# ddiazdom/grlBWT

Measured on NVIDIA B200. Metric: input MB/s through the parse phase of the BCR BWT construction (all grammar rounds on device); whole construction: bwt_total, higher is better.
Workload: dtype u8

## Files before the change

grlbwt_b200/__init__.py:

```python
from .api import (GrlGpu, GrlGpuError, Round, Stats, build_bwt, build_bwt_file, build_bwt_packed, build_bwt_to, invert_rl_bwt, parse_rl_bwt, lib_gpu, lib_host,
                  selftest_compact, selftest_induce, selftest_scan, selftest_sort, FLAG_SMALL_TABLE,
                  FLAG_FORCE_SLOW_SCAN, FLAG_KEEP_DICT, FLAG_FORCE_UNCACHED, FLAG_SMALL_PILOT, FLAG_FORCE_DOUBLING, FLAG_FORCE_WALK,
                  FLAG_FORCE_JUMP, LIB_DIR, Slice)
```

grlbwt_b200/api.py:

```python
from __future__ import annotations

import ctypes as C
import os

import numpy as np

LIB_DIR = os.path.join(os.path.dirname(os.path.abspath(__file__)), "lib")
FLAG_SMALL_TABLE, FLAG_FORCE_SLOW_SCAN, FLAG_KEEP_DICT, FLAG_FORCE_UNCACHED, FLAG_SMALL_PILOT, FLAG_FORCE_DOUBLING = 1, 2, 4, 8, 16, 32
FLAG_FORCE_WALK, FLAG_FORCE_JUMP = 64, 128
CELL = {1: np.uint8, 2: np.uint16, 4: np.uint32, 8: np.uint64}


class GrlGpuError(RuntimeError):
    def __init__(self, status, msg):
        super().__init__(f"grlgpu status {status}: {msg}")
        self.status = status


class Stats(C.Structure):
    _fields_ = [(k, C.c_uint64) for k in ("n_syms", "n_strings", "longest_string", "min_sym", "max_sym", "max_sym_freq", "sep_sym")]


class Round(C.Structure):
    _fields_ = [(k, C.c_uint64) for k in ("round", "n_in", "n_strings", "parse_len", "n_phrases", "dict_syms", "max_freq", "alphabet",
# ... 60 lines not shown
        L.grlgpu_round.argtypes = [vp, C.POINTER(Round)]
        L.grlgpu_fetch_level.argtypes = [vp, vp, vp, vp, vp, vp]
        L.grlgpu_fetch_level_async.argtypes = [vp, vp, vp, vp, vp, vp]
        L.grlgpu_fetch_level32.argtypes = [vp, vp, vp, vp, vp, vp, C.c_int]
        L.grlgpu_fetch_wait.argtypes = [vp]
        L.grlgpu_level_checksum.argtypes = [vp, vp]
        L.grlgpu_fetch_parse.argtypes = [vp, vp]
        L.grlgpu_fetch_str_ptrs.argtypes = [vp, vp]
        L.grlgpu_fetch_dictionary.argtypes = [vp, vp, vp, vp, vp]
        L.grlgpu_strerror.restype = C.c_char_p
        L.grlgpu_strerror.argtypes = [C.c_int]
        L.grlgpu_last_error.restype = C.c_char_p
        L.grlgpu_last_error.argtypes = [vp]
        L.grlgpu_create_on_stream.argtypes = [C.POINTER(vp), C.c_int, u64, vp]
        L.grlgpu_profile_enable.argtypes = [vp, C.c_int]
        L.grlgpu_profile_reset.argtypes = [vp]
        L.grlgpu_launch_count.argtypes = [vp]
        L.grlgpu_launch_count.restype = u64
        L.grlgpu_profile_entry.argtypes = [vp, C.c_int, C.c_char_p, C.c_int, C.POINTER(u64), C.POINTER(C.c_double), C.POINTER(u64)]
        L.grlgpu_histogram.argtypes = [vp, vp]
        L.grlgpu_nccl_unique_id.argtypes = [vp]
        L.grlgpu_comm_create_nccl.argtypes = [C.POINTER(vp), vp, C.c_int, C.c_int, C.c_int]
        L.grlgpu_comm_create_ipc.argtypes = [C.POINTER(vp), C.c_char_p, C.c_int, C.c_int, C.c_int]
        L.grlgpu_can_peer.argtypes = [C.c_int, C.c_int]
        L.grlgpu_local_group_create.argtypes = [C.POINTER(vp), C.c_int]
        L.grlgpu_local_group_abort.argtypes = [vp]
        L.grlgpu_local_group_destroy.argtypes = [vp]
        L.grlgpu_comm_create_local.argtypes = [C.POINTER(vp), vp, C.c_int, C.c_int]
        L.grlgpu_comm_destroy.argtypes = [vp]
        L.grlgpu_comm_info.argtypes = [vp, C.POINTER(u64), C.POINTER(u64), C.POINTER(u64), C.c_char_p, C.c_int]
        L.grlgpu_comm_times.argtypes = [vp, C.POINTER(C.c_double), C.POINTER(C.c_double)]
        L.grlgpu_set_peers.argtypes = [vp, vp, C.c_int]
        L.grlgpu_mg_stats.argtypes = [vp, vp, C.POINTER(Stats)]
        L.grlgpu_mg_round.argtypes = [vp, vp, C.POINTER(Round)]
        L.grlgpu_mg_slice_info.argtypes = [vp, C.POINTER(Slice)]
        L.grlgpu_mg_fetch_slice.argtypes = [vp, vp, vp, vp, vp, vp, C.c_int, C.c_int]
        L.grlgpu_mg_slice_checksum.argtypes = [vp, vp]
        L.grlgpu_text_begin.argtypes = [vp, u64, C.c_int, u64]
        L.grlgpu_text_stage.argtypes = [vp, C.POINTER(vp), C.POINTER(u64)]
        L.grlgpu_text_commit.argtypes = [vp, u64]
        L.grlgpu_text_end.argtypes = [vp]
        L.grlgpu_level_park.argtypes = [vp, C.c_int, vp]
        L.grlgpu_copy_to_host.argtypes = [C.c_int, vp, vp, u64]
        L.grlgpu_invert.argtypes = [vp, vp, u64, C.c_int, u64, vp, u64, C.POINTER(Invert)]
        L.grlgpu_fm_load.argtypes = [vp, vp, u64, C.POINTER(FmInfo)]
        L.grlgpu_fm_count.argtypes = [vp, vp, vp, u64, C.c_int, vp, C.POINTER(FmQuery)]
        L.grlgpu_fm_locate.argtypes = [vp, vp, vp, u64, C.c_int, vp, vp, vp, u64, C.POINTER(FmQuery)]
        L.grlgpu_fm_approx_count.argtypes = [vp, vp, vp, u64, C.c_int, C.c_uint32, vp, vp, vp, u64, C.POINTER(FmApprox)]
        L.grlgpu_fm_approx_locate.argtypes = [vp, vp, vp, u64, C.c_int, C.c_uint32, vp, vp, vp, vp, u64, C.POINTER(FmApprox)]
        L.grlgpu_fm_extract.argtypes = [vp, vp, vp, vp, u64, C.c_int, vp, vp, u64, C.POINTER(FmExtract)]
        L.grlgpu_fm_drop.argtypes = [vp]
        L.grlgpu_selftest_scan.argtypes = [vp, u64, vp, vp]
        L.grlgpu_selftest_sort.argtypes = [vp, vp, u64, C.c_int]
        L.grlgpu_selftest_compact.argtypes = [vp, vp, u64, vp, vp]
        L.grlgpu_selftest_ipc_rendezvous.argtypes = [C.c_char_p, C.c_int, C.c_int, C.c_int]
        _gpu = L
    return _gpu


def lib_host():
    global _host
    if _host is None:
        lib_gpu()
        path = os.path.join(LIB_DIR, "libgrlbwt.so")
        if not os.path.exists(path):
            raise RuntimeError(f"{path} is missing: build it with `make -C grlbwt_b200`")
        L = C.CDLL(path)
        L.grlbwt_build.argtypes = [C.c_void_p, C.c_uint64, C.c_int, C.c_int, C.c_int, C.c_int, C.POINTER(BwtResult)]
        L.grlbwt_free_result.argtypes = [C.POINTER(BwtResult)]
        L.grlbwt_build_file.argtypes = [C.c_char_p, C.c_char_p, C.c_int, C.c_int, C.c_int, C.c_int]
        L.grlbwt_last_error.restype = C.c_char_p
        L.grlbwt_build_mg.argtypes = [C.c_void_p, C.c_uint64, C.c_int, C.c_void_p, C.c_int, C.c_int, C.c_int, C.c_int, C.POINTER(BwtResult)]
        L.grlbwt_build_to.argtypes = [C.c_void_p, C.c_uint64, C.c_int, C.c_void_p, C.c_int, C.c_int, C.c_int, C.c_void_p, C.c_void_p, C.c_uint64, C.POINTER(BwtResult)]
        L.grlbwt_build_packed.argtypes = [C.c_void_p, C.c_uint64, C.c_int, C.c_void_p, C.c_int, C.c_int, C.c_int, C.c_void_p, C.c_uint64, C.POINTER(C.c_uint64),
                                          C.POINTER(BwtResult)]
        L.grlbwt_last_digests.argtypes = [C.c_void_p, C.c_uint64]
        L.grlbwt_last_digests.restype = C.c_uint64
        L.grlbwt_last_exchange_bytes.restype = C.c_uint64
        L.grlbwt_last_comm.restype = C.c_char_p
        _host = L
    return _host


def _ptr(a):
    return None if a is None else a.ctypes.data_as(C.c_void_p)


def _carve(sizes, arena, offset):
    if arena is None:
        return [np.zeros(n, dt) for n, dt in sizes], None
    arrs, off = [], int(offset)
    for n, dt in sizes:
        nb = n * np.dtype(dt).itemsize
        off = (off + 15) & ~15
        if off + nb > arena.size:
            raise GrlGpuError(-1, "fetch arena too small")
        arrs.append(arena[off:off + nb].view(dt))
        off += nb
    return arrs, (off + 15) & ~15


class GrlGpu:

    def __init__(self, device: int = 0, flags: int = 0, stream: int = 0):
        self._L = lib_gpu()
        self._h = C.c_void_p()
# ... 435 lines not shown


def selftest_induce(levels, final_parse: np.ndarray, n_threads: int = 0):
    L = lib_host()
    n = len(levels)
    u64p, u8p = C.POINTER(C.c_uint64), C.POINTER(C.c_uint8)
    keep = []

    def arr(key, dt, ptype):
        out = (ptype * n)()
        for i, lv in enumerate(levels):
            a = np.ascontiguousarray(lv[key], dt)
            if a.size == 0:
                a = np.zeros(1, dt)
            keep.append(a)
            out[i] = a.ctypes.data_as(ptype)
        return out

    alph = np.array([lv["alphabet"] for lv in levels], np.uint64)
    tot = np.array([lv["tot"] for lv in levels], np.uint64)
    npre = np.array([len(lv["pre_sym"]) for lv in levels], np.uint64)
    fp = np.ascontiguousarray(final_parse, np.uint64)
    res = BwtResult()
    L.grlbwt_selftest_induce.argtypes = [C.c_int, C.c_void_p, C.c_void_p, C.POINTER(u64p), C.POINTER(u64p), C.POINTER(u8p), C.c_void_p,
                                         C.POINTER(u64p), C.POINTER(u64p), C.c_void_p, C.c_uint64, C.c_int, C.POINTER(BwtResult)]
    rc = L.grlbwt_selftest_induce(n, _ptr(alph), _ptr(tot), arr("rule_l", np.uint64, u64p), arr("rule_r", np.uint64, u64p),
                                  arr("has_hocc", np.uint8, u8p), _ptr(npre), arr("pre_sym", np.uint64, u64p), arr("pre_len", np.uint64, u64p),
                                  _ptr(fp), fp.size, n_threads, C.byref(res))
    if rc != 0:
        raise RuntimeError(L.grlbwt_last_error().decode())
    try:
        return (np.ctypeslib.as_array(res.syms, shape=(res.n_runs,)).copy(), np.ctypeslib.as_array(res.lens, shape=(res.n_runs,)).copy())
    finally:
        L.grlbwt_free_result(C.byref(res))


def selftest_scan(a: np.ndarray):
    a = np.ascontiguousarray(a, np.uint32)
    out, tot = np.zeros(a.size, np.uint64), np.zeros(1, np.uint64)
    rc = lib_gpu().grlgpu_selftest_scan(_ptr(a), a.size, _ptr(out), _ptr(tot))
    if rc != 0:
        raise GrlGpuError(rc, lib_gpu().grlgpu_strerror(rc).decode())
    return out, int(tot[0])


def selftest_sort(keys: np.ndarray, vals: np.ndarray, n_bits: int):
    k, v = np.ascontiguousarray(keys, np.uint64).copy(), np.ascontiguousarray(vals, np.uint32).copy()
    rc = lib_gpu().grlgpu_selftest_sort(_ptr(k), _ptr(v), k.size, n_bits)
    if rc != 0:
        raise GrlGpuError(rc, lib_gpu().grlgpu_strerror(rc).decode())
    return k, v


def selftest_compact(bits: np.ndarray, prev_bits, n_bits: int):
    b = np.ascontiguousarray(bits, np.uint32)
    pb = None if prev_bits is None else np.ascontiguousarray(prev_bits, np.uint32)
    out, cnt = np.zeros(max(1, n_bits), np.uint64), np.zeros(1, np.uint64)
    rc = lib_gpu().grlgpu_selftest_compact(_ptr(b), _ptr(pb), n_bits, _ptr(out), _ptr(cnt))
    if rc != 0:
        raise GrlGpuError(rc, lib_gpu().grlgpu_strerror(rc).decode())
    return out[: int(cnt[0])]
```

grlbwt_b200/csrc/grlgpu.cu:

```cuda
#include "../../include/grlgpu.h"
#include "util.cuh"
#include "primitives.cuh"
#include "parse_kernels.cuh"
#include "dict_kernels.cuh"
#include "comm.hpp"

#include <algorithm>
#include <cstring>
#include <memory>
#include <vector>

using namespace grl;


struct DevLevel {
    int sym_bytes = 4;
    u64 tot = 0, n_pre = 0;
    DevBuf<u8> rule_l, rule_r, has_hocc, pre_sym;
    DevBuf<u64> pre_len;
    bool present() const { return rule_l.p != nullptr; }
};

struct LevelView {
    int sym_bytes;
// ... 404 lines not shown
               R.einfo.p, (const u32*)voff.p, c->alphabet + 1, R.sym_bits, R.K, R.spare, R.keys.p, R.vals.p);
}

void refine_sort_groups(cudaStream_t st, const u64* nk, const u32* gflag, u64 nA, int key_bits, DevBuf<u32>& perm, DevBuf<u32>& flags) {
    perm.alloc(nA, st);
    flags.alloc(nA, st);
    if (nA == 0) return;
    DevBuf<u32> lflag(nA, st), lexcl(nA, st), cnt(1, st);
    GRL_LAUNCH("ext_local_sort", nA * 24, ext_local_sort_kernel, (unsigned)div_up(nA, LS_WIN), LS_THREADS, 0, st, nk, gflag, nA, perm.p, flags.p, lflag.p);
    exclusive_scan<u32, u32>(lflag.p, lexcl.p, nA, cnt.p, st);
    const u64 nLft = d2h_scalar(cnt.p, st);
    if (getenv("GRLGPU_TRACE")) fprintf(stderr, "[grlgpu]   refine sort: %llu active, %llu through the device-wide path\n", nA, nLft);
    if (nLft == 0) return;
    DevBuf<u32> lpos(nLft, st), lv(nLft, st), lv_alt(nLft, st), lg(nLft, st), gexcl(nLft, st), lf(nLft, st);
    DevBuf<u64> lk(nLft, st), lk_alt(nLft, st), lnk(nLft, st);
    GRL_LAUNCH("ext_left_gather", nA * 8 + nLft * 32, ext_left_gather_kernel, grid_for(nA, 256), 256, 0, st, lflag.p, lexcl.p, nk, gflag, nA, lpos.p, lk.p, lnk.p, lv.p, lg.p);
    exclusive_scan<u32, u32>(lg.p, gexcl.p, nLft, cnt.p, st);
    const u64 n_groups = d2h_scalar(cnt.p, st);
    u64 *kp = lk.p, *ka = lk_alt.p;
    u32 *vp = lv.p, *va = lv_alt.p;
    radix_sort_pairs(&kp, &vp, &ka, &va, nLft, key_bits, st);
    GRL_LAUNCH("ext_gid", nLft * 12, ext_gid_kernel, grid_for(nLft, 256), 256, 0, st, lg.p, gexcl.p, nLft);
    GRL_LAUNCH("ext_group_keys", nLft * 16, ext_group_keys_kernel, grid_for(nLft, 256), 256, 0, st, vp, gexcl.p, nLft, kp);
    radix_sort_pairs(&kp, &vp, &ka, &va, nLft, std::max(1, bit_width64(n_groups)), st);
    GRL_LAUNCH("ext_heads", nLft * 24, ext_heads_kernel, grid_for(nLft, 256), 256, 0, st, vp, kp, lnk.p, nLft, lf.p);
    GRL_LAUNCH("ext_left_scatter", nLft * 20, ext_left_scatter_kernel, grid_for(nLft, 256), 256, 0, st, lpos.p, vp, lf.p, nLft, perm.p, flags.p);
    GRL_CUDA(cudaStreamSynchronize(st));
}

template <class SymT>
void stage_dict(Round& R) {
    grlgpu_ctx* c = R.c;
    cudaStream_t st = R.st;
    const u64 nE = R.nE, A = c->alphabet;
    const SymT* D = (const SymT*)R.D_raw.p;
    IsSuffix isuf{c->is_suffix.p, c->sep, c->first};

    const bool ext_mode = R.ext_mode;
    const u64 nS = R.nS;
    const u64 n_words = div_up(nS, 32);
    DevBuf<u32> order_buf, head_bits(n_words, st);
    u64 G = 0;
    {
        DevBuf<u64> keys = std::move(R.keys), keys_alt(nS, st);
        DevBuf<u32> vals = std::move(R.vals), vals_alt(nS, st);
        const int sym_bits = R.sym_bits, K = R.K;
        if (!ext_mode) {
            keys.alloc(nS, st);
            vals.alloc(nS, st);
            GRL_LAUNCH("sfx_first_key", nE * (sizeof(SymT) + 4 + 12), (sfx_first_key_kernel<SymT>), grid_for(nE, 256), 256, 0, st, D, R.rem.p, nE, A + 1, sym_bits, K, keys.p, vals.p);
        }
        u64 *kp = keys.p, *ka = keys_alt.p;
        u32 *vp = vals.p, *va = vals_alt.p;
        radix_sort_pairs(&kp, &vp, &ka, &va, nS, std::min(64, sym_bits * K + R.spare), st);
        if (vp != vals.p) std::swap(vals, vals_alt);
        order_buf = std::move(vals);
        vals_alt.release();
        u32* order_w = order_buf.p;
        u64 nA = 0;
        DevBuf<u32> apos;
        if (ext_mode) {
            {
                DevBuf<u32> flags(nS, st), active_bits(n_words, st);
                GRL_LAUNCH("first_heads", nS * 12, first_heads_kernel, grid_for(nS, 256), 256, 0, st, kp, nS, sym_bits, R.spare, A + 1, flags.p, head_bits.p, active_bits.p);
                keys.release(); keys_alt.release();
                BitmapCompactor ac;
                nA = ac.count(active_bits.p, nS, st);
                apos.alloc(nA, st);
                if (nA) ac.write<u32>(nullptr, apos.p);
            }
            u64 dpt = (u64)K;
            while (nA > 0) {
                if (dpt > R.max_len + 1) throw Error(GRLGPU_ERR_STATE, "suffix refinement did not converge");
                DevBuf<u64> nk(nA, st);
                DevBuf<u32> ev(nA, st), gflag(nA, st), excl(nA, st), cnt(1, st), perm, flags;
                GRL_LAUNCH("ext_keys", nA * 32, (ext_keys_kernel<SymT>), grid_for(nA, 256), 256, 0, st, apos.p, order_w, D, R.rem.p, head_bits.p, nA, dpt, A + 1, sym_bits, K,
                           (u64*)nullptr, (u32*)nullptr, nk.p, ev.p, gflag.p);
                if (getenv("GRLGPU_TRACE")) fprintf(stderr, "[grlgpu] round %d refine: depth %llu, active %llu (of %llu sorted)\n", c->round + 1, dpt, nA, nS);
                refine_sort_groups(st, nk.p, gflag.p, nA, std::min(64, sym_bits * K), perm, flags);
                const u32* avp = perm.p;
                GRL_LAUNCH("ext_writeback", nA * 16, ext_writeback_kernel, grid_for(nA, 256), 256, 0, st, apos.p, avp, ev.p, flags.p, nA, order_w, head_bits.p);
                dpt += (u64)K;
                GRL_LAUNCH("ext_next", nA * 16, ext_next_kernel, grid_for(nA, 256), 256, 0, st, apos.p, avp, ev.p, head_bits.p, R.rem.p, nA, nS, dpt, flags.p);
                exclusive_scan<u32, u32>(flags.p, excl.p, nA, cnt.p, st);
                const u64 nA2 = d2h_scalar(cnt.p, st);
                DevBuf<u32> apos2(nA2, st);
                if (nA2) GRL_LAUNCH("compact_apos", nA * 12, compact_apos_kernel, grid_for(nA, 256), 256, 0, st, flags.p, excl.p, apos.p, nA, apos2.p);
                apos = std::move(apos2);
                nA = nA2;
            }
        } else {
        R.rank.alloc(nE, st);
        {
            DevBuf<u32> flags(nE, st), excl(nE, st), active_bits(n_words, st), gcount(1, st);
            GRL_LAUNCH("first_heads", nE * 12, first_heads_kernel, grid_for(nE, 256), 256, 0, st, kp, nE, sym_bits, 0, A + 1, flags.p, head_bits.p, active_bits.p);
            keys.release(); keys_alt.release();
            exclusive_scan<u32, u32>(flags.p, excl.p, nE, gcount.p, st);
            const u64 G0 = d2h_scalar(gcount.p, st);
            DevBuf<u32> head_pos(G0, st);
            GRL_LAUNCH("head_pos", nE * 8, head_pos_kernel, grid_for(nE, 256), 256, 0, st, flags.p, excl.p, (const u32*)nullptr, nE, head_pos.p);
            if (nE <= (1ull << 24)) {
                GRL_LAUNCH("assign_hrank", nE * 20, assign_hrank_kernel, grid_for(nE, 256), 256, 0, st, flags.p, excl.p, head_pos.p, order_w, nE, R.rank.p);
            } else {
                DevBuf<u32> pk(nE, st), pv(nE, st), pk2(nE, st), pv2(nE, st);
                GRL_LAUNCH("hrank_pairs", nE * 20, hrank_pairs_kernel, grid_for(nE, 256), 256, 0, st, flags.p, excl.p, head_pos.p, order_w, nE, pk.p, pv.p);
                u32 *k1 = pk.p, *v1 = pv.p, *k2 = pk2.p, *v2 = pv2.p;
                radix_partition_u32(&k1, &v1, &k2, &v2, nE, 24, st);
// ... 1100 lines not shown
    return guarded(ctx, [&] { ctx->fm.reset(); });
}

int grlgpu_profile_enable(grlgpu_ctx* ctx, int on) {
    if (!ctx) return GRLGPU_ERR_ARG;
    ctx->prof.resolve();
    ctx->prof.timing = on != 0;
    return GRLGPU_OK;
}
int grlgpu_profile_reset(grlgpu_ctx* ctx) {
    if (!ctx) return GRLGPU_ERR_ARG;
    ctx->prof.reset();
    return GRLGPU_OK;
}
uint64_t grlgpu_launch_count(const grlgpu_ctx* ctx) { return ctx ? ctx->prof.launches : 0; }
int grlgpu_profile_entry(grlgpu_ctx* ctx, int index, char* name, int name_cap, uint64_t* launches, double* total_ms, uint64_t* model_bytes) {
    if (!ctx || !name || name_cap <= 0) return GRLGPU_ERR_ARG;
    ctx->prof.resolve();
    if (index < 0 || (size_t)index >= ctx->prof.acc.size()) return 1;
    auto it = ctx->prof.acc.begin();
    std::advance(it, index);
    snprintf(name, (size_t)name_cap, "%s", it->first.c_str());
    if (launches) *launches = it->second.launches;
    if (total_ms) *total_ms = it->second.ms;
    if (model_bytes) *model_bytes = it->second.bytes;
    return GRLGPU_OK;
}

const char* grlgpu_strerror(int status) {
    switch (status) {
        case GRLGPU_OK: return "ok";
        case GRLGPU_ERR_ARG: return "invalid argument";
        case GRLGPU_ERR_ILL_FORMED: return "the collection is ill formed";
        case GRLGPU_ERR_CUDA: return "CUDA error or no usable device";
        case GRLGPU_ERR_NOMEM: return "out of device memory";
        case GRLGPU_ERR_STATE: return "call out of order";
        case GRLGPU_ERR_LIMIT: return "size limit of the device path exceeded";
    }
    return "unknown status";
}
const char* grlgpu_last_error(const grlgpu_ctx* ctx) { return ctx ? ctx->last_error.c_str() : t_last_error.c_str(); }

int grlgpu_selftest_scan(const uint32_t* in, uint64_t n, uint64_t* out_exclusive, uint64_t* total) {
    return guarded(nullptr, [&] {
        cudaStream_t st = nullptr;
        DevBuf<u32> din(n, st);
        DevBuf<u64> dout(n, st), tot(1, st);
        GRL_CUDA(cudaMemcpy(din.p, in, n * 4, cudaMemcpyHostToDevice));
        exclusive_scan<u32, u64>(din.p, dout.p, n, tot.p, st);
        GRL_CUDA(cudaMemcpy(out_exclusive, dout.p, n * 8, cudaMemcpyDeviceToHost));
        GRL_CUDA(cudaMemcpy(total, tot.p, 8, cudaMemcpyDeviceToHost));
    });
}
int grlgpu_selftest_sort(uint64_t* keys, uint32_t* vals, uint64_t n, int n_bits) {
    return guarded(nullptr, [&] {
        cudaStream_t st = nullptr;
        DevBuf<u64> k(n, st), ka(n, st);
        DevBuf<u32> v(n, st), va(n, st);
        GRL_CUDA(cudaMemcpy(k.p, keys, n * 8, cudaMemcpyHostToDevice));
        GRL_CUDA(cudaMemcpy(v.p, vals, n * 4, cudaMemcpyHostToDevice));
        u64 *kp = k.p, *kap = ka.p;
        u32 *vp = v.p, *vap = va.p;
        radix_sort_pairs(&kp, &vp, &kap, &vap, n, n_bits, st);
        GRL_CUDA(cudaStreamSynchronize(st));
        GRL_CUDA(cudaMemcpy(keys, kp, n * 8, cudaMemcpyDeviceToHost));
        GRL_CUDA(cudaMemcpy(vals, vp, n * 4, cudaMemcpyDeviceToHost));
    });
}
int grlgpu_selftest_compact(const uint32_t* bits, const uint32_t* prev_bits, uint64_t n_bits, uint64_t* out, uint64_t* count) {
    return guarded(nullptr, [&] {
        cudaStream_t st = nullptr;
        const u64 n_words = div_up(n_bits, 32);
        DevBuf<u32> b(n_words, st), pb(n_words, st);
        GRL_CUDA(cudaMemcpy(b.p, bits, n_words * 4, cudaMemcpyHostToDevice));
        if (prev_bits) GRL_CUDA(cudaMemcpy(pb.p, prev_bits, n_words * 4, cudaMemcpyHostToDevice));
        BitmapCompactor bc;
        const u64 cnt = bc.count(b.p, n_bits, st);
        DevBuf<u64> o(cnt, st);
        bc.write<u64>(prev_bits ? pb.p : nullptr, o.p);
        GRL_CUDA(cudaMemcpy(out, o.p, cnt * 8, cudaMemcpyDeviceToHost));
        *count = cnt;
    });
}

}
```

grlbwt_b200/csrc/primitives.cuh:

```cuda
#pragma once
#include "util.cuh"

namespace grl {

constexpr int SCAN_THREADS = 256;
constexpr int SCAN_ITEMS = 8;
constexpr int SCAN_TILE = SCAN_THREADS * SCAN_ITEMS;

template <class T>
__device__ __forceinline__ void scan_load(const T* in, u64 base, u64 n, bool vec, T (&v)[SCAN_ITEMS]) {
    constexpr int NV = SCAN_ITEMS * sizeof(T) / 16, PER = 16 / sizeof(T);
    if (vec && base + SCAN_ITEMS <= n) {
        const uint4* p = reinterpret_cast<const uint4*>(in + base);
#pragma unroll
        for (int q = 0; q < NV; q++) {
            const uint4 x = p[q];
            memcpy(&v[q * PER], &x, 16);
        }
    } else {
#pragma unroll
        for (int i = 0; i < SCAN_ITEMS; i++) v[i] = (base + i < n) ? in[base + i] : T(0);
    }
}
template <class T>
// ... 258 lines not shown
    {
        const u32 d = threadIdx.x;
        const u64 my_goff = goff[(u64)d * tiles + blockIdx.x];
        u32 c[RS_WARPS], run = 0;
#pragma unroll
        for (int w = 0; w < RS_WARPS; w++) { c[w] = s_cnt[w * 257 + d]; run += c[w]; }
        u32 tot;
        u32 ex = block_exclusive_sum<u32>(run, s_scan, tot);
        s_delta[d] = my_goff - ex;
#pragma unroll
        for (int w = 0; w < RS_WARPS; w++) { s_cnt[w * 257 + d] = ex; ex += c[w]; }
    }
    __syncthreads();
#pragma unroll
    for (int r = 0; r < ITEMS; r++) {
        const u64 idx = tile_base + (u64)warp * WARP_ITEMS + (u64)r * 32 + lane;
        if (idx < n) {
            const u32 d = (u32)(key[r] >> shift) & 255u;
            const u32 pos = wc[d] + rnk[r];
            s_keys[pos] = key[r];
            s_vals[pos] = val[r];
        }
    }
    __syncthreads();
    const u64 rem = n - tile_base;
    const u32 valid = rem < (u64)TILE ? (u32)rem : (u32)TILE;
    for (u32 i = threadIdx.x; i < valid; i += RS_THREADS) {
        const KeyT k = s_keys[i];
        const u32 d = (u32)(k >> shift) & 255u;
        const u64 g = s_delta[d] + i;
        keys_out[g] = k;
        vals_out[g] = s_vals[i];
    }
}

template <class KeyT>
inline void radix_pass(KeyT** keys, u32** vals, KeyT** keys_alt, u32** vals_alt, u64 n, int shift, DevBuf<u32>& hist, DevBuf<u64>& goff, cudaStream_t st) {
    GRL_CUDA(cudaFuncSetAttribute(radix_scatter_kernel<KeyT, RS_ITEMS>, cudaFuncAttributeMaxDynamicSharedMemorySize, (int)rs_smem_bytes<KeyT, RS_ITEMS>()));
    const u64 tiles = div_up(n, RS_THREADS * RS_ITEMS);
    GRL_LAUNCH("radix_hist", n * sizeof(KeyT), (radix_hist_kernel<KeyT, RS_ITEMS>), (unsigned)tiles, RS_THREADS, 0, st, *keys, n, shift, hist.p, tiles);
    exclusive_scan<u32, u64>(hist.p, goff.p, 256 * tiles, nullptr, st);
    GRL_LAUNCH("radix_scatter", n * 2 * (sizeof(KeyT) + 4), (radix_scatter_kernel<KeyT, RS_ITEMS>), (unsigned)tiles, RS_THREADS, (rs_smem_bytes<KeyT, RS_ITEMS>()), st, *keys,
               *vals, *keys_alt, *vals_alt, n, shift, goff.p, tiles);
    KeyT* tk = *keys; *keys = *keys_alt; *keys_alt = tk;
    u32* tv = *vals; *vals = *vals_alt; *vals_alt = tv;
}
inline void radix_sort_pairs(u64** keys, u32** vals, u64** keys_alt, u32** vals_alt, u64 n, int n_bits, cudaStream_t st) {
    if (n <= 1 || n_bits <= 0) return;
    const u64 tiles = div_up(n, RS_THREADS * RS_ITEMS);
    DevBuf<u32> hist(256 * tiles, st);
    DevBuf<u64> goff(256 * tiles, st);
    for (int shift = 0; shift < n_bits; shift += 8) radix_pass<u64>(keys, vals, keys_alt, vals_alt, n, shift, hist, goff, st);
}
inline void radix_partition_u32(u32** keys, u32** vals, u32** keys_alt, u32** vals_alt, u64 n, int shift, cudaStream_t st) {
    const u64 tiles = div_up(n, RS_THREADS * RS_ITEMS);
    DevBuf<u32> hist(256 * tiles, st);
    DevBuf<u64> goff(256 * tiles, st);
    radix_pass<u32>(keys, vals, keys_alt, vals_alt, n, shift, hist, goff, st);
}
inline void radix_sort_pairs_u32(u32** keys, u32** vals, u32** keys_alt, u32** vals_alt, u64 n, int n_bits, cudaStream_t st) {
    if (n <= 1 || n_bits <= 0) return;
    const u64 tiles = div_up(n, RS_THREADS * RS_ITEMS);
    DevBuf<u32> hist(256 * tiles, st);
    DevBuf<u64> goff(256 * tiles, st);
    for (int shift = 0; shift < n_bits; shift += 8) radix_pass<u32>(keys, vals, keys_alt, vals_alt, n, shift, hist, goff, st);
}

static __global__ void reduce_max_u64_kernel(const u64* __restrict__ in, u64 n, u64* out) {
    u64 m = 0;
    for (u64 i = (u64)blockIdx.x * blockDim.x + threadIdx.x; i < n; i += (u64)gridDim.x * blockDim.x) m = in[i] > m ? in[i] : m;
    m = warp_max(m);
    if (lane_id() == 0 && m) atomicMax(out, m);
}

}
```

include/grlgpu.h:

```cpp
#ifndef GRLGPU_H
#define GRLGPU_H
#include <stdint.h>

#ifdef __cplusplus
extern "C" {
#endif

typedef struct grlgpu_ctx grlgpu_ctx;

enum grlgpu_status {
    GRLGPU_OK = 0,
    GRLGPU_ERR_ARG = -1,
    GRLGPU_ERR_ILL_FORMED = -2,
    GRLGPU_ERR_CUDA = -3,
    GRLGPU_ERR_NOMEM = -4,
    GRLGPU_ERR_STATE = -5,
    GRLGPU_ERR_LIMIT = -6
};

#define GRLGPU_FLAG_SMALL_TABLE 1ull
#define GRLGPU_FLAG_FORCE_SLOW_SCAN 2ull
#define GRLGPU_FLAG_FORCE_UNCACHED 8ull
#define GRLGPU_FLAG_SMALL_PILOT 16ull
#define GRLGPU_FLAG_FORCE_DOUBLING 32ull
// ... 126 lines not shown
} grlgpu_fm_extract_t;
int grlgpu_fm_extract(grlgpu_ctx* ctx, const uint32_t* str_id, const uint32_t* from, const uint32_t* len, uint64_t n_req,
                      int cell_bytes, uint64_t* out_off , void* out, uint64_t cap_cells, grlgpu_fm_extract_t* info);

int grlgpu_level_checksum(grlgpu_ctx* ctx, uint64_t* out4);

int grlgpu_fetch_parse(grlgpu_ctx* ctx, void* dst);
int grlgpu_fetch_str_ptrs(grlgpu_ctx* ctx, uint64_t* dst);
int grlgpu_fetch_dictionary(grlgpu_ctx* ctx, uint64_t* syms, uint64_t* lens, uint64_t* freqs, uint64_t* metas);

uint64_t grlgpu_trim(void);

const char* grlgpu_strerror(int status);
const char* grlgpu_last_error(const grlgpu_ctx* ctx);

typedef struct grlgpu_comm grlgpu_comm;
typedef struct grlgpu_local_group grlgpu_local_group;
int grlgpu_nccl_unique_id(void* id128);
int grlgpu_comm_create_nccl(grlgpu_comm** comm, const void* id128, int rank, int world, int device);
int grlgpu_comm_create_ipc(grlgpu_comm** comm, const char* session, int rank, int world, int device);
int grlgpu_local_group_create(grlgpu_local_group** group, int world);
int grlgpu_local_group_abort(grlgpu_local_group* group);
int grlgpu_local_group_destroy(grlgpu_local_group* group);
int grlgpu_comm_create_local(grlgpu_comm** comm, grlgpu_local_group* group, int rank, int device);
int grlgpu_comm_destroy(grlgpu_comm* comm);
int grlgpu_comm_info(const grlgpu_comm* comm, uint64_t* bytes_sent, uint64_t* n_bulk, uint64_t* n_small, char* kind, int kind_cap);
int grlgpu_comm_times(const grlgpu_comm* comm, double* ms_bulk, double* ms_small);
int grlgpu_set_peers(grlgpu_ctx* ctx, const int* devices, int n_devices);
int grlgpu_can_peer(int device_a, int device_b);

int grlgpu_histogram(grlgpu_ctx* ctx, uint64_t* hist256);
int grlgpu_mg_stats(grlgpu_ctx* ctx, grlgpu_comm* comm, grlgpu_stats_t* global_out);
int grlgpu_mg_round(grlgpu_ctx* ctx, grlgpu_comm* comm, grlgpu_round_t* out);

typedef struct {
    uint64_t rank_base, tot_local;
    uint64_t pre_first, n_pre_local;
    uint64_t exchange_bytes;
    uint64_t n_in_local, parse_len_local;
    uint32_t sym_bytes;
    uint32_t reserved;
} grlgpu_slice_t;
int grlgpu_mg_slice_info(grlgpu_ctx* ctx, grlgpu_slice_t* out);
int grlgpu_mg_fetch_slice(grlgpu_ctx* ctx, void* rule_l, void* rule_r, uint8_t* has_hocc, void* pre_sym, void* pre_len, int len_bytes, int async);
int grlgpu_mg_slice_checksum(grlgpu_ctx* ctx, uint64_t* out4);

int grlgpu_profile_enable(grlgpu_ctx* ctx, int on);
int grlgpu_profile_reset(grlgpu_ctx* ctx);
uint64_t grlgpu_launch_count(const grlgpu_ctx* ctx);
int grlgpu_profile_entry(grlgpu_ctx* ctx, int index, char* name, int name_cap, uint64_t* launches, double* total_ms, uint64_t* model_bytes);

int grlgpu_selftest_scan(const uint32_t* in, uint64_t n, uint64_t* out_exclusive, uint64_t* total);
int grlgpu_selftest_sort(uint64_t* keys, uint32_t* vals, uint64_t n, int n_bits);
int grlgpu_selftest_compact(const uint32_t* bits, const uint32_t* prev_bits, uint64_t n_bits, uint64_t* out, uint64_t* count);
int grlgpu_selftest_ipc_rendezvous(const char* session, int rank, int world, int rounds);

#ifdef __cplusplus
}
#endif
#endif
```

Before: 11040.

## Sort suffix keys MSD-first: top-bit radix passes then per-bucket on-chip sort

Replaces the full LSD radix sort of suffix keys with a hybrid. It first runs global radix passes on the top 24 bits only. Buckets of up to 2048 items are then finished inside shared memory within per-tile windows, and larger buckets are gathered into a side array, radix-sorted on bucket id plus low bits, and scattered back. This aims to cut the number of full-array global passes when keys are wide, at the cost of several extra small kernels, a host sync for bucket statistics, and more complex code with edge cases around bucket and tile boundaries.

```diff
diff --git a/grlbwt_b200/__init__.py b/grlbwt_b200/__init__.py
--- a/grlbwt_b200/__init__.py
+++ b/grlbwt_b200/__init__.py
@@ -1,4 +1,4 @@
 from .api import (GrlGpu, GrlGpuError, Round, Stats, build_bwt, build_bwt_file, build_bwt_packed, build_bwt_to, invert_rl_bwt, parse_rl_bwt, lib_gpu, lib_host,
-                  selftest_compact, selftest_induce, selftest_scan, selftest_sort, FLAG_SMALL_TABLE,
+                  selftest_compact, selftest_induce, selftest_scan, selftest_sort, selftest_sort_topfirst, FLAG_SMALL_TABLE,
                   FLAG_FORCE_SLOW_SCAN, FLAG_KEEP_DICT, FLAG_FORCE_UNCACHED, FLAG_SMALL_PILOT, FLAG_FORCE_DOUBLING, FLAG_FORCE_WALK,
                   FLAG_FORCE_JUMP, LIB_DIR, Slice)
diff --git a/grlbwt_b200/api.py b/grlbwt_b200/api.py
--- a/grlbwt_b200/api.py
+++ b/grlbwt_b200/api.py
@@ -136,6 +136,7 @@
         L.grlgpu_fm_drop.argtypes = [vp]
         L.grlgpu_selftest_scan.argtypes = [vp, u64, vp, vp]
         L.grlgpu_selftest_sort.argtypes = [vp, vp, u64, C.c_int]
+        L.grlgpu_selftest_sort_topfirst.argtypes = [vp, vp, u64, C.c_int]
         L.grlgpu_selftest_compact.argtypes = [vp, vp, u64, vp, vp]
         L.grlgpu_selftest_ipc_rendezvous.argtypes = [C.c_char_p, C.c_int, C.c_int, C.c_int]
         _gpu = L
@@ -677,6 +678,14 @@
     return k, v
 
 
+def selftest_sort_topfirst(keys: np.ndarray, vals: np.ndarray, n_bits: int):
+    k, v = np.ascontiguousarray(keys, np.uint64).copy(), np.ascontiguousarray(vals, np.uint32).copy()
+    rc = lib_gpu().grlgpu_selftest_sort_topfirst(_ptr(k), _ptr(v), k.size, n_bits)
+    if rc != 0:
+        raise GrlGpuError(rc, lib_gpu().grlgpu_strerror(rc).decode())
+    return k, v
+
+
 def selftest_compact(bits: np.ndarray, prev_bits, n_bits: int):
     b = np.ascontiguousarray(bits, np.uint32)
     pb = None if prev_bits is None else np.ascontiguousarray(prev_bits, np.uint32)
diff --git a/grlbwt_b200/csrc/grlgpu.cu b/grlbwt_b200/csrc/grlgpu.cu
--- a/grlbwt_b200/csrc/grlgpu.cu
+++ b/grlbwt_b200/csrc/grlgpu.cu
@@ -480,7 +480,7 @@
         }
         u64 *kp = keys.p, *ka = keys_alt.p;
         u32 *vp = vals.p, *va = vals_alt.p;
-        radix_sort_pairs(&kp, &vp, &ka, &va, nS, std::min(64, sym_bits * K + R.spare), st);
+        radix_sort_pairs_topfirst(&kp, &vp, &ka, &va, nS, std::min(64, sym_bits * K + R.spare), st);
         if (vp != vals.p) std::swap(vals, vals_alt);
         order_buf = std::move(vals);
         vals_alt.release();
@@ -1687,7 +1687,7 @@
         GRL_CUDA(cudaMemcpy(total, tot.p, 8, cudaMemcpyDeviceToHost));
     });
 }
-int grlgpu_selftest_sort(uint64_t* keys, uint32_t* vals, uint64_t n, int n_bits) {
+static int selftest_sort_with(uint64_t* keys, uint32_t* vals, uint64_t n, int n_bits, void (*sort)(u64**, u32**, u64**, u32**, u64, int, cudaStream_t)) {
     return guarded(nullptr, [&] {
         cudaStream_t st = nullptr;
         DevBuf<u64> k(n, st), ka(n, st);
@@ -1696,11 +1696,15 @@
         GRL_CUDA(cudaMemcpy(v.p, vals, n * 4, cudaMemcpyHostToDevice));
         u64 *kp = k.p, *kap = ka.p;
         u32 *vp = v.p, *vap = va.p;
-        radix_sort_pairs(&kp, &vp, &kap, &vap, n, n_bits, st);
+        sort(&kp, &vp, &kap, &vap, n, n_bits, st);
         GRL_CUDA(cudaStreamSynchronize(st));
         GRL_CUDA(cudaMemcpy(keys, kp, n * 8, cudaMemcpyDeviceToHost));
         GRL_CUDA(cudaMemcpy(vals, vp, n * 4, cudaMemcpyDeviceToHost));
     });
+}
+int grlgpu_selftest_sort(uint64_t* keys, uint32_t* vals, uint64_t n, int n_bits) { return selftest_sort_with(keys, vals, n, n_bits, radix_sort_pairs); }
+int grlgpu_selftest_sort_topfirst(uint64_t* keys, uint32_t* vals, uint64_t n, int n_bits) {
+    return selftest_sort_with(keys, vals, n, n_bits, radix_sort_pairs_topfirst);
 }
 int grlgpu_selftest_compact(const uint32_t* bits, const uint32_t* prev_bits, uint64_t n_bits, uint64_t* out, uint64_t* count) {
     return guarded(nullptr, [&] {
diff --git a/grlbwt_b200/csrc/primitives.cuh b/grlbwt_b200/csrc/primitives.cuh
--- a/grlbwt_b200/csrc/primitives.cuh
+++ b/grlbwt_b200/csrc/primitives.cuh
@@ -334,6 +334,233 @@
     DevBuf<u64> goff(256 * tiles, st);
     for (int shift = 0; shift < n_bits; shift += 8) radix_pass<u64>(keys, vals, keys_alt, vals_alt, n, shift, hist, goff, st);
 }
+constexpr int TF_TOP_BITS = 24;
+constexpr int TF_THREADS = 512, TF_WARPS = TF_THREADS / 32;
+constexpr u32 TF_TILE = 2048, TF_BIG = 2048;
+constexpr u32 TF_CAP = TF_TILE + TF_BIG;
+constexpr int TF_ITEMS = TF_CAP / TF_THREADS;
+static_assert(TF_BIG >= TF_TILE, "at most one big bucket may start in a tile");
+static_assert(TF_CAP <= 65536, "window positions are 16-bit");
+constexpr size_t tf_smem_bytes() { return (size_t)TF_CAP * 2 * (sizeof(u64) + sizeof(u16)) + (size_t)TF_WARPS * 257 * sizeof(u32) + 36 * sizeof(u32); }
+
+static __global__ void __launch_bounds__(256) tf_heads_kernel(const u64* __restrict__ keys, u64 n, int s, u32* __restrict__ head_bits) {
+    const u64 i = (u64)blockIdx.x * blockDim.x + threadIdx.x;
+    const bool h = i < n && (i == 0 || (keys[i] >> s) != (keys[i - 1] >> s));
+    const u32 w = __ballot_sync(0xffffffffu, h);
+    if (lane_id() == 0 && i < n) head_bits[i >> 5] = w;
+}
+
+static __global__ void __launch_bounds__(256) tf_buckets_kernel(const u64* __restrict__ bstart, u64 nbk, u64 n, u64 n_tiles, u32* __restrict__ big_flag,
+                                                                u64* __restrict__ big_size, u32* __restrict__ tile_lo, u64* __restrict__ stats) {
+    const u64 j = (u64)blockIdx.x * blockDim.x + threadIdx.x;
+    if (j > nbk) return;
+    const u64 p = j < nbk ? bstart[j] : n;
+    const u64 t_min = j == 0 ? 0 : bstart[j - 1] / TF_TILE + 1, t_max = j < nbk ? p / TF_TILE : n_tiles;
+    for (u64 t = t_min; t <= t_max; t++) tile_lo[t] = (u32)j;
+    if (j == nbk) return;
+    const u64 sz = (j + 1 < nbk ? bstart[j + 1] : n) - p;
+    big_flag[j] = sz > TF_BIG;
+    big_size[j] = sz > TF_BIG ? sz : 0;
+    atomicMax(stats + 2, sz);
+}
+
+static __global__ void __launch_bounds__(256) tf_big_list_kernel(const u64* __restrict__ bstart, const u32* __restrict__ big_flag, const u64* __restrict__ big_idx,
+                                                                 const u64* __restrict__ big_size, const u64* __restrict__ side_off, u64 nbk,
+                                                                 u64* __restrict__ bb_start, u64* __restrict__ bb_off) {
+    const u64 j = (u64)blockIdx.x * blockDim.x + threadIdx.x;
+    if (j >= nbk) return;
+    if (big_flag[j]) { bb_start[big_idx[j]] = bstart[j]; bb_off[big_idx[j]] = side_off[j]; }
+    if (j == nbk - 1) bb_off[big_idx[j] + big_flag[j]] = side_off[j] + big_size[j];
+}
+
+__device__ __forceinline__ u64 tf_side_pos(const u64* __restrict__ bb_start, const u64* __restrict__ bb_off, u64 n_big, u64 q, u64& b) {
+    u64 lo = 0, hi = n_big;
+    while (hi - lo > 1) {
+        const u64 mid = (lo + hi) >> 1;
+        if (bb_off[mid] <= q) lo = mid; else hi = mid;
+    }
+    b = lo;
+    return bb_start[lo] + (q - bb_off[lo]);
+}
+static __global__ void __launch_bounds__(256) tf_side_gather_kernel(const u64* __restrict__ keys, const u32* __restrict__ vals, const u64* __restrict__ bb_start,
+                                                                    const u64* __restrict__ bb_off, u64 n_big, u64 n_side, int s, u64* __restrict__ sk, u32* __restrict__ sv) {
+    const u64 q = (u64)blockIdx.x * blockDim.x + threadIdx.x;
+    if (q >= n_side) return;
+    u64 b;
+    const u64 p = tf_side_pos(bb_start, bb_off, n_big, q, b);
+    sk[q] = (b << s) | (keys[p] & ((1ULL << s) - 1ULL));
+    sv[q] = vals[p];
+}
+static __global__ void __launch_bounds__(256) tf_side_scatter_kernel(u64* __restrict__ keys, u32* __restrict__ vals, const u64* __restrict__ bb_start,
+                                                                     const u64* __restrict__ bb_off, u64 n_big, u64 n_side, int s, const u64* __restrict__ sk,
+                                                                     const u32* __restrict__ sv) {
+    const u64 q = (u64)blockIdx.x * blockDim.x + threadIdx.x;
+    if (q >= n_side) return;
+    u64 b;
+    const u64 p = tf_side_pos(bb_start, bb_off, n_big, q, b);
+    const u64 low = (1ULL << s) - 1ULL;
+    keys[p] = (keys[p] & ~low) | (sk[q] & low);
+    vals[p] = sv[q];
+}
+
+__device__ void tf_window_sort(u64* __restrict__ keys, u32* __restrict__ vals, u64 g0, u32 m, int nb, unsigned char* smem) {
+    u64* s_key = (u64*)smem;
+    u16* s_idx = (u16*)(s_key + 2 * TF_CAP);
+    u32* s_cnt = (u32*)(s_idx + 2 * TF_CAP);
+    u32* s_scan = s_cnt + TF_WARPS * 257;
+    u64* s_mask = (u64*)(s_scan + 34);
+    const u32 lane = lane_id(), warp = threadIdx.x >> 5;
+    __syncthreads();
+    if (threadIdx.x == 0) *s_mask = 0;
+    for (u32 q = threadIdx.x; q < m; q += TF_THREADS) { s_key[q] = keys[g0 + q]; s_idx[q] = (u16)q; }
+    __syncthreads();
+    const u64 k0 = s_key[0];
+    u64 diff = 0;
+    for (u32 q = threadIdx.x; q < m; q += TF_THREADS) diff |= s_key[q] ^ k0;
+    diff = __reduce_or_sync(0xffffffffu, (u32)diff) | ((u64)__reduce_or_sync(0xffffffffu, (u32)(diff >> 32)) << 32);
+    if (lane == 0 && diff) atomicOr((unsigned long long*)s_mask, diff);
+    __syncthreads();
+    const u64 mask = *s_mask & (nb >= 64 ? ~0ULL : (1ULL << nb) - 1ULL);
+    if (mask == 0) return;
+    const u32 rounds = (m + TF_WARPS * 32 - 1) / (TF_WARPS * 32), seg = rounds * 32;
+    int cur = 0;
+    for (int sh = 0; sh < nb; sh += 8) {
+        if (((mask >> sh) & 255u) == 0) continue;
+        const u64* ki = s_key + cur * TF_CAP;
+        const u16* ii = s_idx + cur * TF_CAP;
+        for (int i = threadIdx.x; i < TF_WARPS * 257; i += TF_THREADS) s_cnt[i] = 0;
+        __syncthreads();
+        u32* wc = s_cnt + warp * 257;
+        u64 key[TF_ITEMS];
+        u32 rnk[TF_ITEMS];
+#pragma unroll
+        for (int r = 0; r < TF_ITEMS; r++) {
+            if ((u32)r < rounds) {
+                const u32 q = warp * seg + (u32)r * 32 + lane;
+                const bool ok = q < m;
+                key[r] = ok ? ki[q] : 0;
+                const u32 d = ok ? ((u32)(key[r] >> sh) & 255u) : 256u;
+                const u32 mm = __match_any_sync(0xffffffffu, d);
+                const u32 b = wc[d];
+                __syncwarp();
+                if (lane == (u32)(__ffs(mm) - 1)) wc[d] = b + __popc(mm);
+                __syncwarp();
+                rnk[r] = b + __popc(mm & lanemask_lt());
+            }
+        }
+        __syncthreads();
+        {
+            const u32 d = threadIdx.x;
+            u32 c[TF_WARPS], run = 0;
+            if (d < 256) {
+#pragma unroll
+                for (int w = 0; w < TF_WARPS; w++) { c[w] = s_cnt[w * 257 + d]; run += c[w]; }
+            }
+            u32 tot;
+            u32 ex = block_exclusive_sum<u32>(run, s_scan, tot);
+            if (d < 256) {
+#pragma unroll
+                for (int w = 0; w < TF_WARPS; w++) { s_cnt[w * 257 + d] = ex; ex += c[w]; }
+            }
+        }
+        __syncthreads();
+        u64* ko = s_key + (cur ^ 1) * TF_CAP;
+        u16* io = s_idx + (cur ^ 1) * TF_CAP;
+#pragma unroll
+        for (int r = 0; r < TF_ITEMS; r++) {
+            const u32 q = warp * seg + (u32)r * 32 + lane;
+            if ((u32)r < rounds && q < m) {
+                const u32 pos = wc[(u32)(key[r] >> sh) & 255u] + rnk[r];
+                ko[pos] = key[r];
+                io[pos] = ii[q];
+            }
+        }
+        __syncthreads();
+        cur ^= 1;
+    }
+    u32* s_val = (u32*)(s_key + (cur ^ 1) * TF_CAP);
+    for (u32 q = threadIdx.x; q < m; q += TF_THREADS) s_val[q] = vals[g0 + q];
+    __syncthreads();
+    for (u32 q = threadIdx.x; q < m; q += TF_THREADS) {
+        keys[g0 + q] = s_key[cur * TF_CAP + q];
+        vals[g0 + q] = s_val[s_idx[cur * TF_CAP + q]];
+    }
+}
+
+static __global__ void __launch_bounds__(TF_THREADS, 2) tf_finish_kernel(u64* __restrict__ keys, u32* __restrict__ vals, u64 n, const u64* __restrict__ bstart, u64 nbk,
+                                                                          const u32* __restrict__ tile_lo, const u32* __restrict__ big_flag, int nb) {
+    extern __shared__ __align__(16) unsigned char tf_smem[];
+    __shared__ u32 s_big;
+    const u32 lo = tile_lo[blockIdx.x], hi = tile_lo[blockIdx.x + 1];
+    if (lo == hi) return;
+    if (threadIdx.x == 0) s_big = hi;
+    __syncthreads();
+    for (u32 j = lo + threadIdx.x; j < hi; j += TF_THREADS)
+        if (big_flag[j]) s_big = j;
+    __syncthreads();
+    const u32 big = s_big;
+    auto start = [&](u32 j) { return j < nbk ? bstart[j] : n; };
+    if (big > lo) tf_window_sort(keys, vals, bstart[lo], (u32)(start(big) - bstart[lo]), nb, tf_smem);
+    if (big + 1 < hi) tf_window_sort(keys, vals, bstart[big + 1], (u32)(start(hi) - bstart[big + 1]), nb, tf_smem);
+}
+
+inline void radix_sort_pairs_topfirst(u64** keys, u32** vals, u64** keys_alt, u32** vals_alt, u64 n, int n_bits, cudaStream_t st) {
+    const int nb = std::min(64, (n_bits + 7) / 8 * 8);
+    if (n <= 1 || nb <= TF_TOP_BITS) { radix_sort_pairs(keys, vals, keys_alt, vals_alt, n, n_bits, st); return; }
+    const int s = nb - TF_TOP_BITS;
+    const bool trace = getenv("GRLGPU_TRACE") != nullptr;
+    std::chrono::steady_clock::time_point t0;
+    if (trace) { GRL_CUDA(cudaStreamSynchronize(st)); t0 = std::chrono::steady_clock::now(); }
+    {
+        const u64 tiles = div_up(n, RS_THREADS * RS_ITEMS);
+        DevBuf<u32> hist(256 * tiles, st);
+        DevBuf<u64> goff(256 * tiles, st);
+        for (int shift = s; shift < nb; shift += 8) radix_pass<u64>(keys, vals, keys_alt, vals_alt, n, shift, hist, goff, st);
+    }
+    DevBuf<u64> bstart;
+    u64 nbk = 0;
+    {
+        DevBuf<u32> head_bits(div_up(n, 32), st);
+        GRL_LAUNCH("tf_heads", n * 8 + n / 8, tf_heads_kernel, (unsigned)div_up(n, 256), 256, 0, st, *keys, n, s, head_bits.p);
+        BitmapCompactor bc;
+        nbk = bc.count(head_bits.p, n, st);
+        bstart.alloc(nbk, st);
+        bc.write<u64>(nullptr, bstart.p);
+    }
+    const u64 n_tiles = div_up(n, TF_TILE);
+    DevBuf<u32> big_flag(nbk, st), tile_lo(n_tiles + 1, st);
+    DevBuf<u64> big_size(nbk, st), big_idx(nbk, st), side_off(nbk, st), stats(3, st);
+    stats.zero();
+    GRL_LAUNCH("tf_buckets", nbk * 24 + n_tiles * 4, tf_buckets_kernel, (unsigned)div_up(nbk + 1, 256), 256, 0, st, bstart.p, nbk, n, n_tiles, big_flag.p, big_size.p,
+               tile_lo.p, stats.p);
+    exclusive_scan<u32, u64>(big_flag.p, big_idx.p, nbk, stats.p, st);
+    exclusive_scan<u64, u64>(big_size.p, side_off.p, nbk, stats.p + 1, st);
+    u64 h[3];
+    d2h_small(h, stats.p, sizeof h, st);
+    const u64 n_big = h[0], n_side = h[1];
+    GRL_CUDA(cudaFuncSetAttribute(tf_finish_kernel, cudaFuncAttributeMaxDynamicSharedMemorySize, (int)tf_smem_bytes()));
+    GRL_LAUNCH("tf_finish", (n - n_side) * 24 + n_tiles * 8, tf_finish_kernel, (unsigned)n_tiles, TF_THREADS, tf_smem_bytes(), st, *keys, *vals, n, bstart.p, nbk, tile_lo.p,
+               big_flag.p, nb);
+    if (n_side) {
+        DevBuf<u64> bb_start(n_big, st), bb_off(n_big + 1, st), sk_alt(n_side, st);
+        DevBuf<u32> sv_alt(n_side, st);
+        GRL_LAUNCH("tf_big_list", nbk * 28, tf_big_list_kernel, (unsigned)div_up(nbk, 256), 256, 0, st, bstart.p, big_flag.p, big_idx.p, big_size.p, side_off.p, nbk, bb_start.p, bb_off.p);
+        u64 *sk = *keys_alt, *ska = sk_alt.p;
+        u32 *sv = *vals_alt, *sva = sv_alt.p;
+        GRL_LAUNCH("tf_side_gather", n_side * 24, tf_side_gather_kernel, (unsigned)div_up(n_side, 256), 256, 0, st, *keys, *vals, bb_start.p, bb_off.p, n_big, n_side, s, sk, sv);
+        DevBuf<u32> hist(256 * div_up(n_side, RS_THREADS * RS_ITEMS), st);
+        DevBuf<u64> goff(256 * div_up(n_side, RS_THREADS * RS_ITEMS), st);
+        const int side_bits = s + bit_width64(n_big - 1);
+        for (int shift = 0; shift < side_bits; shift += 8) radix_pass<u64>(&sk, &sv, &ska, &sva, n_side, shift, hist, goff, st);
+        GRL_LAUNCH("tf_side_scatter", n_side * 36, tf_side_scatter_kernel, (unsigned)div_up(n_side, 256), 256, 0, st, *keys, *vals, bb_start.p, bb_off.p, n_big, n_side, s, sk, sv);
+    }
+    if (trace) {
+        GRL_CUDA(cudaStreamSynchronize(st));
+        fprintf(stderr, "[grlgpu] sort topfirst: n %llu, %d bits, T %d, %llu buckets, largest %llu, %llu items on chip, %llu in %llu big buckets, %.2f ms\n", n, nb,
+                TF_TOP_BITS, nbk, h[2], n - n_side, n_side, n_big, std::chrono::duration<double, std::milli>(std::chrono::steady_clock::now() - t0).count());
+    }
+}
+
 inline void radix_partition_u32(u32** keys, u32** vals, u32** keys_alt, u32** vals_alt, u64 n, int shift, cudaStream_t st) {
     const u64 tiles = div_up(n, RS_THREADS * RS_ITEMS);
     DevBuf<u32> hist(256 * tiles, st);
diff --git a/include/grlgpu.h b/include/grlgpu.h
--- a/include/grlgpu.h
+++ b/include/grlgpu.h
@@ -202,6 +202,7 @@
 
 int grlgpu_selftest_scan(const uint32_t* in, uint64_t n, uint64_t* out_exclusive, uint64_t* total);
 int grlgpu_selftest_sort(uint64_t* keys, uint32_t* vals, uint64_t n, int n_bits);
+int grlgpu_selftest_sort_topfirst(uint64_t* keys, uint32_t* vals, uint64_t n, int n_bits);
 int grlgpu_selftest_compact(const uint32_t* bits, const uint32_t* prev_bits, uint64_t n_bits, uint64_t* out, uint64_t* count);
 int grlgpu_selftest_ipc_rendezvous(const char* session, int rank, int world, int rounds);
 
```

New measurement: 9756 (median of 6 runs). 0.884x the previous value.
